# happykygo/GNN-eCommerce

Hardware: AMD Instinct MI355X
Metric: edges propagated/sec per LGConv layer (higher is better)
Workload: dtype f32; 1 GPU; configs[1]: 1639358 users x 54571 items, 20314816 directed edges, 3 LGConv layers, emb_dim 64, get_embedding (K hops + fused layer sum); parallelism=single, seed=0

## Files before the change

### gnn-ecommerce_amd/_native.py

```python
from __future__ import annotations

import ctypes
import os
from ctypes import CFUNCTYPE, POINTER, Structure, c_char_p, c_float, c_int, c_int32, c_int64, c_size_t, c_uint64, c_void_p
from typing import Optional

import torch

LIB_NAME = "liblgconv_hip.so"
LIB_PATH = os.environ.get("LGCN_LIB_PATH") or os.path.join(os.path.dirname(os.path.abspath(__file__)), "csrc", LIB_NAME)
ABI_VERSION = 14

ST_INDEX_OOB = 1
ST_SAMPLER_EXHAUSTED = 2

class SweepCfg(Structure):
    _fields_ = [("n_bands", c_int32), ("waves_per_band_round", c_int32), ("row_cap", c_int32), ("piece_cap", c_int32),
                ("lookahead", c_int32), ("groups", c_int32), ("round_order", c_int32)]


class SweepDims(Structure):
    _fields_ = [("n_bands", c_int32), ("rounds", c_int32), ("row_cap", c_int32), ("piece_cap", c_int32),
                ("n_rows", c_int32), ("groups", c_int32),
                ("n_waves", c_int64), ("n_slabs", c_int64), ("n_slots", c_int64), ("n_entries", c_int64),
# ... 71 lines not shown
    "lgc_sweep_dplan_free": (None, [c_void_p]),
    "lgc_sweep_ok": (c_int, [c_int32, c_int64, c_int64]),
    "lgc_spmm_sweep": (c_int, [c_void_p, c_void_p, c_void_p, c_void_p, c_int64, c_int32, c_int32, c_void_p, c_int32, c_void_p,
                               c_int32, c_void_p, c_int64, c_void_p, c_int64, c_void_p, c_int64, c_void_p, c_int64, c_float, c_float,
                               c_int32, c_void_p]),
    "lgc_apply_route": (c_int, [POINTER(OperatorC), c_int64, c_int64, c_int64, c_int64, c_int32]),
    "lgc_apply": (c_int, [POINTER(OperatorC), c_int64, c_void_p, c_int64, c_void_p, c_int64, c_void_p, c_int64, c_float, c_float,
                          c_int32, c_void_p]),
    "lgc_hop_exchange": (c_int, [POINTER(OperatorC), POINTER(OperatorC), c_int64, c_void_p, c_int64, c_void_p, c_int64, c_void_p,
                                 c_int64, c_float, c_float, c_int32, c_int32, c_int32, c_int32, EXCHANGE_FN, c_void_p, c_void_p]),
    "lgc_segment_sum": (c_int, [c_void_p, c_void_p, c_void_p, c_void_p, c_int64, c_float, c_void_p, c_int64, c_int64, c_int32,
                                c_int32, c_void_p]),
    "lgc_pair_dot_rows": (c_int, [c_void_p, c_int64, c_int32, c_int64, c_void_p, c_void_p, c_int64, c_void_p, c_void_p, c_void_p,
                                  c_void_p, c_void_p, c_void_p]),
    "lgc_reg_rows": (c_int, [c_void_p, c_int64, c_int32, c_int64, c_void_p, c_int64, c_void_p, c_int64, c_void_p, c_int64, c_float,
                             c_void_p, c_void_p, c_void_p, c_void_p]),
    "lgc_bpr_loss": (c_int, [c_void_p, c_void_p, c_int64, c_int64, c_void_p, c_void_p, c_void_p]),
    "lgc_pair_seed_vals": (c_int, [c_void_p, c_void_p, c_void_p, c_void_p, c_void_p, c_int64, c_int32, c_void_p, c_void_p]),
    "lgc_seed_prepare": (c_int, [c_void_p, c_int64, c_int64, c_int64, c_void_p, c_void_p, c_void_p, c_void_p, c_void_p, c_void_p,
                                 c_void_p, c_void_p, c_void_p]),
    "lgc_seed_flags": (c_int, [c_void_p, c_int64, c_int64, c_void_p, c_int32, c_void_p]),
    "lgc_seed_pull": (c_int, [c_void_p, c_void_p, c_int32, c_int32, c_int32, c_void_p, c_int32, c_void_p, c_int32, c_void_p,
                              c_void_p, c_void_p, c_void_p, c_void_p, c_int64, c_int64, c_void_p, c_int64, c_int32, c_void_p]),
    "lgc_seed_mark": (c_int, [c_void_p, c_void_p, c_int32, c_int32, c_void_p, c_int64, c_void_p, c_int64, c_int32, c_void_p]),
    "lgc_adam_step": (c_int, [c_void_p, c_void_p, c_void_p, c_void_p, c_int64, c_float, c_float, c_float, c_float, c_float,
                              c_float, c_void_p]),
    "lgc_adam_step_hp": (c_int, [c_void_p, c_void_p, c_void_p, c_void_p, c_int64, c_void_p, c_void_p]),
    "lgc_lincomb": (c_int, [c_void_p, c_int64, c_void_p, c_void_p, c_void_p, c_int32, c_int64, c_int32, c_void_p]),
    "lgc_mask_topk": (c_int, [c_void_p, c_int64, c_void_p, c_int64, c_void_p, c_void_p, c_void_p, c_int64, c_int32, c_int32,
                              c_void_p, c_void_p, c_void_p]),
    "lgc_fold_in": (c_int, [c_void_p, c_void_p, c_void_p, c_int64, c_void_p, c_void_p, c_int64, c_int64, c_void_p, c_void_p,
                            c_int64, c_int64, c_float, c_int32, c_int32, c_void_p, c_int64, c_void_p, c_void_p]),
    "lgc_score_rows": (c_int, [c_void_p, c_int64, c_int64, c_void_p, c_int64, c_void_p, c_int64, c_int32, c_int32, c_void_p,
                               c_int64, c_void_p, c_void_p]),
    "lgc_topk_hits": (c_int, [c_void_p, c_int64, c_int32, c_void_p, c_void_p, c_void_p, c_int64, c_int64, c_void_p, c_void_p,
                              c_void_p, c_void_p]),
    "lgc_metric_sums": (c_int, [c_void_p, c_void_p, c_int64, c_void_p, c_void_p, c_void_p]),
    "lgc_rank_metrics": (c_int, [c_void_p, c_int64, c_int32, c_void_p, c_void_p, c_void_p, c_void_p, c_int64, c_int64,
                                 POINTER(c_int32), c_int32, c_void_p, c_void_p, c_void_p, c_void_p, c_void_p]),
    "lgc_column_sums": (c_int, [c_void_p, c_int64, c_int64, c_int32, c_void_p, c_void_p]),
    "lgc_topk_coverage": (c_int, [c_void_p, c_int64, c_int32, c_int64, POINTER(c_int32), c_int32, c_int64, c_void_p, c_void_p,
                                  c_void_p, c_void_p]),
    "lgc_bfs_init": (c_int, [c_void_p, c_int32, c_int64, c_void_p, c_void_p, c_void_p, c_void_p]),
    "lgc_bfs_level": (c_int, [c_void_p, c_void_p, c_int32, c_int32, c_int32, c_void_p, c_int32, c_uint64, c_void_p, c_void_p,
                              c_void_p, c_void_p, c_void_p]),
    "lgc_bfs_resolve": (c_int, [c_void_p, c_void_p, c_int32, c_int64, c_int64, c_void_p, c_int32, c_void_p, c_void_p, c_void_p,
                                c_void_p]),
    "lgc_bfs_backtrack": (c_int, [c_void_p, c_void_p, c_int64, c_void_p, c_int32, c_void_p, c_void_p, c_int32, c_int64,
                                  c_void_p, c_int32, c_void_p]),
    "lgc_sample_triples": (c_int, [c_void_p, c_int64, c_void_p, c_void_p, c_void_p, c_void_p, c_int64, c_int64, c_uint64,
                                   c_uint64, c_void_p, c_void_p, c_void_p, c_void_p]),
    "lgc_pair_dot": (c_int, [c_void_p, c_int64, c_int32, c_int64, c_void_p, c_void_p, c_int64, c_void_p,
                             c_void_p, c_void_p]),
}


class NativeLibraryError(RuntimeError):
    """The HIP library is missing, stale, or a call into it failed."""


_lib: Optional[ctypes.CDLL] = None


def load() -> ctypes.CDLL:
    global _lib
    if _lib is not None:
        return _lib
    if not os.path.isfile(LIB_PATH):
        raise NativeLibraryError(
            f"{LIB_PATH} not found: the MI355X propagation library has not been built. "
            "Run `python -c 'import __graft_entry__ as g; g.build()'` (or `make -C gnn-ecommerce_amd/csrc`). "
            "There is no CPU or PyTorch fallback for this path.")
    try:
        lib = ctypes.CDLL(LIB_PATH)
    except OSError as exc:
        raise NativeLibraryError(f"cannot load {LIB_PATH}: {exc}") from exc
    for name, (restype, argtypes) in SIGNATURES.items():
        try:
            fn = getattr(lib, name)
        except AttributeError as exc:
            raise NativeLibraryError(f"{LIB_PATH} does not export {name}; rebuild it") from exc
        fn.restype, fn.argtypes = restype, argtypes
    if lib.lgc_abi_version() != ABI_VERSION:
        raise NativeLibraryError(f"{LIB_PATH} has ABI {lib.lgc_abi_version()}, expected {ABI_VERSION}; rebuild it")
    _lib = lib
    return lib


def check(code: int, what: str) -> None:
    if code != 0:
        text = load().lgc_error_string(code).decode()
        raise NativeLibraryError(f"{what} failed: {text} (code {code})")


def ptr(t: Optional[torch.Tensor]) -> Optional[int]:
    return None if t is None else t.data_ptr()


def stream_of(device: torch.device) -> int:
    return torch.cuda.current_stream(device).cuda_stream


def require_device(t: torch.Tensor, name: str) -> None:
    if not t.is_cuda:
        raise NativeLibraryError(
            f"{name} is on {t.device}: the LightGCN propagation path runs only on a ROCm device "
# ... 36 lines not shown
```

### gnn-ecommerce_amd/graph.py

```python
from __future__ import annotations

import os
from collections import OrderedDict
from dataclasses import dataclass, field
from typing import Dict, List, Optional, Tuple

import torch
from torch import Tensor

from . import _native

SHORT_MAX = int(os.environ.get("LGCN_SHORT_MAX", "32"))
CHUNK_LEN = int(os.environ.get("LGCN_CHUNK_LEN", "256"))
USER_CHUNK_LEN = int(os.environ.get("LGCN_USER_CHUNK_LEN", "4096"))
TILE_WIDTHS = (8, 16, 32)
USE_TILES = os.environ.get("LGCN_TILES", "1") == "1"
TILES_PER_WAVE = int(os.environ.get("LGCN_TILES_PER_WAVE", "1"))
TILE_ORDER = os.environ.get("LGCN_TILE_ORDER", "cold")
USE_SWEEP = os.environ.get("LGCN_SWEEP", "auto")
SWEEP_MIN_ENTRIES = int(os.environ.get("LGCN_SWEEP_MIN_ENTRIES", "1000000"))
SWEEP_ADAPTIVE_BANDS = os.environ.get("LGCN_SWEEP_ADAPTIVE_BANDS", "1") == "1"
SWEEP_PIECE_ENTRIES = int(os.environ.get("LGCN_SWEEP_PIECE_ENTRIES", "20"))
SWEEP_CFG = dict(n_bands=int(os.environ.get("LGCN_SWEEP_BANDS", "8")), waves_per_band_round=int(os.environ.get("LGCN_SWEEP_WAVES", "256")),
                 row_cap=int(os.environ.get("LGCN_SWEEP_ROW_CAP", "78")),
# ... 537 lines not shown

def _rows_split_scratch(device: torch.device, n_ids: int, dim: int) -> Tuple[Tensor, Tensor]:
    import threading
    key = (device, torch.cuda.current_stream(device).cuda_stream, threading.get_ident(), dim)
    got = _rows_scratch.get(key)
    if got is None or got[0].numel() < n_ids + 2:
        cap = max(n_ids, 4096)
        got = (torch.empty(cap + 2, dtype=torch.int32, device=device),
               torch.empty((cap + ROWS_SPLIT_ROOM, dim), dtype=torch.float32, device=device))
        _rows_scratch[key] = got
    return got


def apply_rows(op: "Operator", rows: Tensor, x: Tensor, out: Tensor, a: float = 1.0, r: Optional[Tensor] = None,
               b: float = 0.0, split: bool = False, compact: bool = False) -> Tensor:
    _check_table(x, "x")
    _check_table(out, "out")
    if r is not None:
        _check_table(r, "r")
    _native.require_device(rows, "rows")
    if rows.dtype != torch.int64 or rows.dim() != 1:
        raise TypeError("rows must be a 1-D int64 tensor")
    dim = x.size(1)
    if out.size(1) != dim or (r is not None and r.size(1) != dim):
        raise ValueError("x, out and r must have the same width")
    if compact and not split:
        raise ValueError("compact output needs split=True")
    rows = rows.contiguous()
    lib = _native.load()
    p = op.plan
    n_ids = rows.numel()
    with torch.cuda.device(x.device):
        if split:
            if n_ids == 0:
                return out
            if out.size(0) < (n_ids if compact else p.row_end):
                raise ValueError("out has too few rows")
            work, partials = _rows_split_scratch(x.device, n_ids, dim)
            code = lib.lgc_spmm_rows_split(_native.ptr(op.rowptr), _native.ptr(op.entries), p.row_begin, p.row_end, _native.ptr(rows),
                                           n_ids, x.size(0), _native.ptr(x), x.stride(0), _native.ptr(out), out.stride(0),
                                           out.size(0), _native.ptr(r), 0 if r is None else r.stride(0), float(a), float(b), dim,
                                           int(compact), _native.ptr(work), _native.ptr(partials), partials.size(0),
                                           _native.stream_of(x.device))
            _native.check(code, "lgc_spmm_rows_split")
            return out
        code = lib.lgc_spmm_rows(_native.ptr(op.rowptr), _native.ptr(op.entries), p.row_begin, p.row_end, _native.ptr(rows),
                                 n_ids, min(x.size(0), out.size(0)), _native.ptr(x), x.stride(0), _native.ptr(out),
                                 out.stride(0), _native.ptr(r), 0 if r is None else r.stride(0), float(a), float(b), dim,
                                 _native.stream_of(x.device))
    _native.check(code, "lgc_spmm_rows")
    return out


def sweep_choice(lib, dim: int, table_rows: int, stride: int) -> int:
    sweep = int(lib.lgc_sweep_ok(dim, table_rows, stride))
    return 0 if (sweep == 2 and not SWEEP_WIDE) else sweep


def _check_table(t: Tensor, name: str) -> None:
    _native.require_device(t, name)
    if t.dtype != torch.float32 or t.dim() != 2 or t.stride(1) != 1:
        raise TypeError(f"{name} must be a 2-D fp32 tensor with unit inner stride, got {t.dtype} {tuple(t.shape)}")


class PropGraph:

    def __init__(self, edge_index: Tensor, edge_weight: Optional[Tensor], num_nodes: int,
                 normalize: bool = True, short_max: int = SHORT_MAX, chunk_len: int = CHUNK_LEN,
                 keep_edge_values: bool = False):
        _native.require_device(edge_index, "edge_index")
        if edge_index.dtype != torch.int64 or edge_index.dim() != 2 or edge_index.size(0) != 2:
            raise TypeError("edge_index must be an int64 tensor of shape [2, E]")
        if edge_weight is not None:
            _native.require_device(edge_weight, "edge_weight")
            if edge_weight.dtype != torch.float32 or edge_weight.shape != (edge_index.size(1),):
                raise TypeError("edge_weight must be fp32 of shape [E]")
            if edge_weight.device != edge_index.device:
                raise RuntimeError("edge_index and edge_weight must be on the same device")
        self.device = edge_index.device
        self.num_nodes = int(num_nodes)
        self.num_edges = int(edge_index.size(1))
        self.normalize = bool(normalize)
        self.short_max, self.chunk_len = short_max, chunk_len
        self._key_refs = (edge_index, edge_weight)
        self._edge_index = edge_index.contiguous()
        self._edge_weight = None if edge_weight is None else edge_weight.contiguous()
        self.status = torch.zeros(4, dtype=torch.int32, device=self.device)
        self.deg = torch.empty(self.num_nodes, dtype=torch.float32, device=self.device)
        self.dis = torch.empty(self.num_nodes, dtype=torch.float32, device=self.device)
        self.edge_values = (torch.empty(self.num_edges, dtype=torch.float32, device=self.device)
                            if keep_edge_values else None)
        self.forward_op = self._build(by_source=False)
        self._transpose_op: Optional[Operator] = None
        self.split = self._find_bipartite_split()
        self._halves = {}

    def _build(self, by_source: bool, row_range: Optional[Tuple[int, int]] = None) -> Operator:
        lib = _native.load()
        n, e = self.num_nodes, self.num_edges
        ws_bytes = lib.lgc_build_workspace_bytes(n, e)
        if ws_bytes == 0:
            raise _native.NativeLibraryError("graph too large for int32 indexing")
        ws = torch.empty(ws_bytes, dtype=torch.uint8, device=self.device)
        rowptr = torch.empty(n + 1, dtype=torch.int32, device=self.device)
        entries = torch.empty((e, 2), dtype=torch.int32, device=self.device)
        first = not by_source
        with torch.cuda.device(self.device):
            code = lib.lgc_build_csr(
                _native.ptr(self._edge_index), _native.ptr(self._edge_weight), n, e,
                int(by_source), int(self.normalize),
                None if (first or not self.normalize) else _native.ptr(self.dis),
                _native.ptr(rowptr), _native.ptr(entries),
                _native.ptr(self.edge_values) if first else None,
                _native.ptr(self.deg) if first else None, _native.ptr(self.dis) if first else None,
                _native.ptr(ws), ws_bytes, _native.ptr(self.status), _native.stream_of(self.device))
        _native.check(code, "lgc_build_csr")
        if int(self.status[0].item()) & _native.ST_INDEX_OOB:
            raise IndexError(f"edge_index contains node ids outside [0, {n})")
        lo, hi = row_range if row_range is not None else (0, n)
        return Operator.build(n, rowptr, entries, lo, hi, self.short_max, self.chunk_len)

    def _find_bipartite_split(self) -> Optional[int]:
        if self.num_edges == 0:
            return None
        out = torch.empty(2, dtype=torch.int64, device=self.device)
        lib = _native.load()
        with torch.cuda.device(self.device):
            code = lib.lgc_bipartite_split(_native.ptr(self._edge_index), self.num_edges, _native.ptr(out),
                                           _native.stream_of(self.device))
        _native.check(code, "lgc_bipartite_split")
        lo, hi = out.tolist()
        return lo + 1 if lo < hi else None

    def halves(self, transpose: bool = False) -> Tuple[Operator, Operator]:
        if self.split is None:
            raise ValueError("graph is not bipartite")
        got = self._halves.get(transpose)
        if got is None:
            op = self.transpose_op if transpose else self.forward_op
            got = tuple(Operator.build(op.n_rows, op.rowptr, op.entries, lo, hi, self.short_max, chunk, sweep_cols=cols)
                        for (lo, hi), cols, chunk in (((0, self.split), (self.split, self.num_nodes),
                                                       max(self.chunk_len, USER_CHUNK_LEN)),
                                                      ((self.split, self.num_nodes), (0, self.split), self.chunk_len)))
            self._halves[transpose] = got
        return got

    def prepare(self, dim: int, table_rows: Optional[int] = None, transpose: bool = False) -> "PropGraph":
        lib = _native.load()
        rows = self.num_nodes if table_rows is None else int(table_rows)
        stride = dim if dim % 32 == 0 else (dim + 31) // 32 * 32
        ops = self.halves(transpose) if self.split is not None else ((self.transpose_op if transpose else self.forward_op),)
        import time
        for op in ops:
            t0 = time.perf_counter()
            if op.tiled and dim >= 4:
                op.tiles
            if PLAN_TIMING:
                torch.cuda.synchronize(self.device)
                print(f"[plan] rows [{op.plan.row_begin}, {op.plan.row_end}): tile classes {time.perf_counter() - t0:.3f} s", flush=True)
            t0 = time.perf_counter()
            if op.sweep_cols is not None:
                groups = sweep_choice(lib, dim, rows, stride)
                if groups:
                    op.sweep_plan(groups)
            if PLAN_TIMING:
                torch.cuda.synchronize(self.device)
                print(f"[plan] rows [{op.plan.row_begin}, {op.plan.row_end}): sweep plan total {time.perf_counter() - t0:.3f} s", flush=True)
        torch.cuda.synchronize(self.device)
        return self

    @property
    def transpose_op(self) -> Operator:
        if self._transpose_op is None:
            if self._edge_index is None:
                raise _native.NativeLibraryError("this graph was loaded from a file without its COO: the transposed "
                                                 "operator (backward pass) needs a graph built from edge_index")
            self._transpose_op = self._build(by_source=True)
        return self._transpose_op

    def save(self, path: str, extra: Optional[Dict[str, Tensor]] = None, meta: Optional[Dict[str, str]] = None) -> None:
        from safetensors.torch import save_file
        op = self.forward_op
        tensors = {"rowptr": op.rowptr, "entries": op.entries, "deg": self.deg, "dis": self.dis}
        for k, v in (extra or {}).items():
            tensors["extra." + k] = v
        meta = {**{"user." + k: str(v) for k, v in (meta or {}).items()},
                "format": "lgcn-graph-2", "num_nodes": str(self.num_nodes), "num_edges": str(self.num_edges),
                "normalize": str(int(self.normalize)), "split": "" if self.split is None else str(self.split)}
        save_file({k: v.detach().cpu().contiguous() for k, v in tensors.items()}, path, metadata=meta)

    @staticmethod
    def validate_csr(rowptr: Tensor, entries: Tensor, deg: Tensor, dis: Tensor, num_nodes: int, num_edges: int,
                     split: Optional[int], where: str) -> None:
        def bad(msg):
            raise ValueError(f"{where}: {msg}")
        if num_nodes < 0 or num_edges < 0 or num_nodes >= 2 ** 31 - 1 or num_edges >= 2 ** 31 - 1:
            bad("node or edge count out of range")
        if rowptr.dtype != torch.int32 or rowptr.shape != (num_nodes + 1,):
            bad(f"rowptr must be int32 [{num_nodes + 1}], got {rowptr.dtype} {tuple(rowptr.shape)}")
        if entries.dtype != torch.int32 or entries.shape != (num_edges, 2):
            bad(f"entries must be int32 [{num_edges}, 2], got {entries.dtype} {tuple(entries.shape)}")
        for name, t in (("deg", deg), ("dis", dis)):
            if t.dtype != torch.float32 or t.shape != (num_nodes,):
                bad(f"{name} must be fp32 [{num_nodes}], got {t.dtype} {tuple(t.shape)}")
        if split is not None and not 0 < split < num_nodes:
            bad(f"bipartite split {split} outside (0, {num_nodes})")
# ... 91 lines not shown
```

### gnn-ecommerce_amd/propagate.py

```python
from __future__ import annotations

import os
from typing import List, Optional, Sequence

import torch
from torch import Tensor
from torch.autograd.function import once_differentiable

from . import _native
from .graph import Operator, PropGraph, apply_rows


HOP_EVENT_LOG: Optional[list] = None


def _timed_apply(op: Operator, x: Tensor, out: Tensor, **kw) -> None:
    if HOP_EVENT_LOG is None:
        op.apply(x, out, **kw)
        return
    start, end = torch.cuda.Event(enable_timing=True), torch.cuda.Event(enable_timing=True)
    start.record()
    op.apply(x, out, **kw)
    end.record()
    HOP_EVENT_LOG.append((start, end))


def scratch_table(like: Tensor) -> Tensor:
    n, d = like.shape
    if PAD_INTERNAL and d % 32 != 0:
        stride = (d + 31) // 32 * 32
        return torch.empty((n, stride), dtype=like.dtype, device=like.device)[:, :d]
    return torch.empty_like(like)


PAD_INTERNAL = os.environ.get("LGCN_PAD_INTERNAL", "1") == "1"


def horner_hops(op: Operator, x0: Tensor, alphas: Sequence[float]) -> Tensor:
    k = len(alphas) - 1
    if k == 0:
        return x0 * alphas[0]
    x0 = x0.contiguous()
    h = torch.empty_like(x0) if k == 1 else scratch_table(x0)
    _timed_apply(op, x0, h, a=alphas[k], r=x0, b=alphas[k - 1])
    for layer in range(k - 2, -1, -1):
        nxt = torch.empty_like(x0) if layer == 0 else scratch_table(x0)
        _timed_apply(op, h, nxt, a=1.0, r=x0, b=alphas[layer])
        h = nxt
    return h


USE_BIPARTITE = os.environ.get("LGCN_BIPARTITE", "1") == "1"

class _HopSpan:

    def __enter__(self):
        self.log = HOP_EVENT_LOG
        if self.log is not None:
            self.start, self.end = torch.cuda.Event(enable_timing=True), torch.cuda.Event(enable_timing=True)
            self.start.record()
        return self

    def __exit__(self, *exc):
        if self.log is not None:
            self.end.record()
            self.log.append((self.start, self.end))


def bipartite_sum(user_op: Operator, item_op: Operator, split: int, x0: Tensor, alphas: Sequence[float],
                  final_rows: Optional[Tensor] = None) -> Tensor:
    k = len(alphas) - 1
    if k == 0:
        return x0 * alphas[0]
    x0 = x0.contiguous()
    n = x0.size(0)
    tables = [x0]
    uniform = UNIFORM_ALPHA_SHORTCUT and all(a == alphas[0] for a in alphas) and (UNIFORM_ALPHA_SHORTCUT == "force" or x0.size(1) % 32 == 0)
    for layer in range(1, k + 1):
        with _HopSpan():
            nxt = scratch_table(x0)
            if layer < k:
                item_op.apply(tables[-1], nxt)
                user_op.apply(tables[-1], nxt)
                tables.append(nxt)
            else:
                out = torch.empty_like(x0)
                rows_only = final_rows is not None
                if rows_only and SCORED_ITEM_ROWS_ONLY and item_op.listed_rows_pay(final_rows.numel()):
                    mix = nxt
                    _native.lincomb(mix[split:], [(alphas[l], tables[l - 1][split:]) for l in range(1, k + 1)])
                    if all(a == alphas[0] for a in alphas):
                        rest = mix
                    else:
                        rest = scratch_table(x0)
                        _native.lincomb(rest[split:], [(alphas[l], tables[l][split:]) for l in range(0, k)])
                    apply_rows(item_op, final_rows, tables[-1], out, a=alphas[k], r=rest, b=1.0, split=True)
                elif uniform:
                    mix = nxt
                    _native.lincomb(mix[split:], [(alphas[l], tables[l - 1][split:]) for l in range(1, k + 1)])
                    item_op.apply(tables[-1], out, a=alphas[k], r=mix, b=1.0)
                else:
                    item_op.apply(tables[-1], nxt)
                    tables.append(nxt)
                    mix = scratch_table(x0)
                    _native.lincomb(mix[split:], [(alphas[l], tables[l - 1][split:]) for l in range(1, k + 1)])
                    _native.lincomb(out[split:], [(alphas[l], tables[l][split:]) for l in range(0, k + 1)])
                if not rows_only:
                    user_op.apply(mix, out, a=1.0, r=x0, b=alphas[0])
                else:
                    apply_rows(user_op, final_rows, mix, out, a=1.0, r=x0, b=alphas[0])
    return out


def _layer_sum(graph: PropGraph, x: Tensor, alphas: tuple, transpose: bool, final_rows: Optional[Tensor] = None) -> Tensor:
    if USE_BIPARTITE and graph.split is not None and len(alphas) - 1 <= _native.MAX_TERMS - 1:
        user_op, item_op = graph.halves(transpose)
        return bipartite_sum(user_op, item_op, graph.split, x, alphas, final_rows if SCORED_ROWS_ONLY else None)
    return horner_hops(graph.transpose_op if transpose else graph.forward_op, x, alphas)


UNIFORM_ALPHA_SHORTCUT = {"0": False, "force": "force"}.get(os.environ.get("LGCN_UNIFORM_ALPHA_SHORTCUT", "1"), True)
SCORED_ROWS_ONLY = os.environ.get("LGCN_SCORED_ROWS_ONLY", "1") == "1"
SCORED_ITEM_ROWS_ONLY = os.environ.get("LGCN_SCORED_ITEM_ROWS_ONLY", "1") == "1"


class _PropagateSum(torch.autograd.Function):
    @staticmethod
    def forward(ctx, x0: Tensor, graph: PropGraph, alphas: tuple) -> Tensor:
        ctx.graph, ctx.alphas = graph, alphas
        return _layer_sum(graph, x0.detach(), alphas, transpose=False)

    @staticmethod
    @once_differentiable
    def backward(ctx, grad_out: Tensor):
        return _layer_sum(ctx.graph, grad_out.contiguous(), ctx.alphas, transpose=True), None, None


class _Hop(torch.autograd.Function):

    @staticmethod
    def forward(ctx, x: Tensor, graph: PropGraph) -> Tensor:
        ctx.graph = graph
        x = x.detach().contiguous()
        return graph.forward_op.apply(x, torch.empty_like(x))

    @staticmethod
    @once_differentiable
    def backward(ctx, grad_out: Tensor):
        g = grad_out.contiguous()
        return ctx.graph.transpose_op.apply(g, torch.empty_like(g)), None


def propagate_sum(x0: Tensor, graph: PropGraph, alphas: Sequence[float]) -> Tensor:
    _native.require_device(x0, "embedding table")
    return _PropagateSum.apply(x0, graph, tuple(float(a) for a in alphas))


def hop(x: Tensor, graph: PropGraph) -> Tensor:
    _native.require_device(x, "x")
    return _Hop.apply(x, graph)


_status_words = {}


def _status(device: torch.device) -> Tensor:
    t = _status_words.get(device)
    if t is None:
        t = torch.zeros(4, dtype=torch.int32, device=device)
        _status_words[device] = t
# ... 1001 lines not shown
```

### include/lgconv_hip.h

```cpp
#ifndef LGCONV_HIP_H
#define LGCONV_HIP_H

#include <stddef.h>
#include <stdint.h>

#ifdef __cplusplus
extern "C" {
#endif

#define LGC_ABI_VERSION 14

#define LGC_E_INVAL      (-1)
#define LGC_E_DIM        (-2)
#define LGC_E_WORKSPACE  (-3)
#define LGC_E_RANGE      (-4)
#define LGC_E_ALIGN      (-5)

#define LGC_ST_INDEX_OOB 1

typedef struct lgc_entry {
    int32_t col;
    float   val;
} lgc_entry;

// ... 215 lines not shown
                int32_t normalize, int32_t dim, float *out, int64_t out_stride, int32_t *status, void *stream);

int lgc_score_rows(const float *users, int64_t user_stride, int64_t n_user_rows, const int64_t *row_ids,
                   int64_t n_rows, const float *items, int64_t item_stride, int32_t n_items, int32_t dim,
                   float *out, int64_t out_stride, int32_t *status, void *stream);

int lgc_topk_hits(const int64_t *topk, int64_t topk_stride, int32_t k, const int64_t *pos_ptr,
                  const int64_t *pos_items, const int64_t *list_rows, int64_t n_rows, int64_t n_users,
                  int32_t *hits, double *recall, int32_t *status, void *stream);

int lgc_metric_sums(const int32_t *hits, const double *recall, int64_t n_rows, int64_t *hits_sum,
                    double *recall_sum, void *stream);

#define LGC_RM_PRECISION 0
#define LGC_RM_RECALL    1
#define LGC_RM_NDCG      2
#define LGC_RM_AP        3
#define LGC_RM_RR        4
#define LGC_RM_HIT       5
#define LGC_RM_COUNT     6
#define LGC_RM_MAX_CUTOFFS 8
int lgc_rank_metrics(const int64_t *topk, int64_t topk_stride, int32_t k, const int64_t *pos_ptr,
                     const int64_t *pos_items, const int64_t *pos_distinct, const int64_t *list_rows, int64_t n_rows,
                     int64_t n_users, const int32_t *cutoffs, int32_t n_cut, uint64_t *hit_bits, int32_t *hits,
                     double *metrics, int32_t *status, void *stream);

#define LGC_COLUMN_SUMS_MAX 64
int lgc_column_sums(const double *in, int64_t in_stride, int64_t n_rows, int32_t n_cols, double *out, void *stream);

int lgc_topk_coverage(const int64_t *topk, int64_t topk_stride, int32_t k, int64_t n_rows, const int32_t *cutoffs,
                      int32_t n_cut, int64_t n_items, uint32_t *bitmap, int64_t *counts, int32_t *status, void *stream);

#define LGC_BFS_MAX_SOURCES 64
#define LGC_BFS_UNSET (-3)
int lgc_bfs_init(const int64_t *sources, int32_t n_sources, int64_t n_nodes, uint64_t *seen, uint64_t *frontier,
                 int32_t *status, void *stream);
int lgc_bfs_level(const int32_t *rowptr, const lgc_entry *entries, int32_t row_begin, int32_t row_end, int32_t short_max,
                  const lgc_chunk *chunks, int32_t n_chunks, uint64_t active, const uint64_t *frontier_in,
                  uint64_t *frontier_out, uint64_t *seen, uint64_t *counters, void *stream);
int lgc_bfs_resolve(const int64_t *sources, const int64_t *targets, int32_t n_sources, int64_t n_targets, int64_t n_nodes,
                    const uint64_t *frontier, int32_t level, int32_t *dist, uint64_t *counters, int32_t *status,
                    void *stream);
int lgc_bfs_backtrack(const int32_t *rowptr, const lgc_entry *entries, int64_t n_nodes, const uint64_t *levels,
                      int32_t n_levels, const int64_t *targets, const int32_t *dist, int32_t n_sources, int64_t n_targets,
                      int64_t *paths, int32_t path_len, void *stream);

#define LGC_ST_SAMPLER_EXHAUSTED 2
int lgc_sample_triples(const int64_t *users, int64_t n,
                       const int32_t *pos_ptr, const int64_t *pos_items,
                       const int32_t *ign_ptr, const int64_t *ign_items,
                       int64_t n_users, int64_t n_items, uint64_t seed, uint64_t step,
                       int64_t *pos_out, int64_t *neg_out, int32_t *status, void *stream);

#ifdef __cplusplus
}
#endif
#endif
```

Before: 38.97 billion edges/s.

## Eliminate low-degree users via precomputed item-item Gram operator in bipartite propagation

```diff
diff --git a/gnn-ecommerce_amd/_native.py b/gnn-ecommerce_amd/_native.py
--- a/gnn-ecommerce_amd/_native.py
+++ b/gnn-ecommerce_amd/_native.py
@@ -147,6 +147,15 @@
                                    c_uint64, c_void_p, c_void_p, c_void_p, c_void_p]),
     "lgc_pair_dot": (c_int, [c_void_p, c_int64, c_int32, c_int64, c_void_p, c_void_p, c_int64, c_void_p,
                              c_void_p, c_void_p]),
+    "lgc_reduce_workspace_bytes": (c_size_t, [c_int64, c_int64]),
+    "lgc_reduce_count": (c_int, [c_void_p, c_void_p, c_int64, c_int64, c_int64, c_int32, c_void_p, c_size_t, c_void_p, c_void_p,
+                                 c_void_p]),
+    "lgc_reduce_fill": (c_int, [c_void_p, c_void_p, c_int64, c_int64, c_int64, c_void_p, c_void_p, c_int64, c_int64, c_void_p,
+                                c_void_p, c_void_p]),
+    "lgc_reduce_gram_workspace_bytes": (c_size_t, [c_int64]),
+    "lgc_reduce_gram_count": (c_int, [c_void_p, c_void_p, c_int64, c_int64, c_int64, c_void_p, c_int64, c_void_p, c_size_t,
+                                      c_void_p, c_void_p]),
+    "lgc_reduce_gram_fill": (c_int, [c_void_p, c_int64, c_int64, c_int64, c_int64, c_void_p, c_void_p, c_void_p]),
 }
 
 
diff --git a/gnn-ecommerce_amd/csrc/lgconv_reduce.hip b/gnn-ecommerce_amd/csrc/lgconv_reduce.hip
--- /dev/null
+++ b/gnn-ecommerce_amd/csrc/lgconv_reduce.hip
@@ -0,0 +1,362 @@
+#include "lgconv_common.h"
+
+#include <hipcub/hipcub.hpp>
+
+namespace {
+
+inline size_t r_align_up(size_t v, size_t a) { return (v + a - 1) / a * a; }
+
+struct ReduceWs {
+    int32_t *incount;
+    int32_t *keep_scan;
+    int32_t *ent_scan;
+    long long *pair_scan;
+    void *cub;
+    size_t cub_bytes;
+};
+
+size_t reduce_ws(void *base, int64_t n_nodes, int64_t n_edges, ReduceWs *ws) {
+    size_t cb32 = 0, cb64 = 0;
+    int32_t *n32 = nullptr;
+    long long *n64 = nullptr;
+    const int64_t longest = std::max<int64_t>(n_edges, n_nodes) + 1;
+    (void)hipcub::DeviceScan::ExclusiveSum(nullptr, cb32, n32, n32, (int)longest, (hipStream_t)0);
+    (void)hipcub::DeviceScan::ExclusiveSum(nullptr, cb64, n64, n64, (int)longest, (hipStream_t)0);
+    const size_t cb = std::max(cb32, cb64);
+    const uintptr_t p = reinterpret_cast<uintptr_t>(base);
+    size_t off = 0;
+    auto take = [&](size_t bytes) { const size_t at = off; off += r_align_up(bytes, 256); return p + at; };
+    const uintptr_t a_in = take((size_t)(n_nodes + 1) * 4), a_keep = take((size_t)(n_nodes + 1) * 4),
+                    a_ent = take((size_t)(n_edges + 1) * 4), a_pair = take((size_t)(n_edges + 1) * 8), a_cub = take(cb);
+    if (ws) {
+        ws->incount = reinterpret_cast<int32_t *>(a_in);
+        ws->keep_scan = reinterpret_cast<int32_t *>(a_keep);
+        ws->ent_scan = reinterpret_cast<int32_t *>(a_ent);
+        ws->pair_scan = reinterpret_cast<long long *>(a_pair);
+        ws->cub = reinterpret_cast<void *>(a_cub);
+        ws->cub_bytes = cb;
+    }
+    return off + 256;
+}
+
+struct GramWs {
+    unsigned long long *keys_in, *keys_out;
+    double *vals_in, *vals_out;
+    int32_t *head_scan;
+    void *cub;
+    size_t cub_bytes;
+};
+
+size_t gram_ws(void *base, int64_t n_pairs, GramWs *ws) {
+    size_t cb_sort = 0, cb_scan = 0;
+    unsigned long long *nk = nullptr;
+    double *nv = nullptr;
+    int32_t *n32 = nullptr;
+    const int64_t n = std::max<int64_t>(n_pairs, 1);
+    (void)hipcub::DeviceRadixSort::SortPairs(nullptr, cb_sort, nk, nk, nv, nv, (int)n, 0, 64, (hipStream_t)0);
+    (void)hipcub::DeviceScan::ExclusiveSum(nullptr, cb_scan, n32, n32, (int)(n + 1), (hipStream_t)0);
+    const size_t cb = std::max(cb_sort, cb_scan);
+    const uintptr_t p = reinterpret_cast<uintptr_t>(base);
+    size_t off = 0;
+    auto take = [&](size_t bytes) { const size_t at = off; off += r_align_up(bytes, 256); return p + at; };
+    const uintptr_t a_ki = take((size_t)n * 8), a_ko = take((size_t)n * 8), a_vi = take((size_t)n * 8), a_vo = take((size_t)n * 8),
+                    a_hs = take((size_t)(n + 1) * 4), a_cub = take(cb);
+    if (ws) {
+        ws->keys_in = reinterpret_cast<unsigned long long *>(a_ki);
+        ws->keys_out = reinterpret_cast<unsigned long long *>(a_ko);
+        ws->vals_in = reinterpret_cast<double *>(a_vi);
+        ws->vals_out = reinterpret_cast<double *>(a_vo);
+        ws->head_scan = reinterpret_cast<int32_t *>(a_hs);
+        ws->cub = reinterpret_cast<void *>(a_cub);
+        ws->cub_bytes = cb;
+    }
+    return off + 256;
+}
+
+__device__ inline int32_t row_of_entry(const int32_t *__restrict__ rowptr, int32_t n_rows, int32_t e) {
+    int32_t lo = 0, hi = n_rows;
+    while (hi - lo > 1) {
+        const int32_t mid = lo + (hi - lo) / 2;
+        if (rowptr[mid] <= e) lo = mid; else hi = mid;
+    }
+    return lo;
+}
+
+__global__ void k_reduce_incount(const int32_t *__restrict__ rowptr, const lgc_entry *__restrict__ entries, int32_t n_nodes,
+                                 int32_t split, int32_t n_edges, int32_t *__restrict__ incount) {
+    const int32_t e_begin = max(rowptr[split], 0), e_end = min(rowptr[n_nodes], n_edges);
+    for (int64_t e = e_begin + (int64_t)blockIdx.x * blockDim.x + threadIdx.x; e < e_end; e += (int64_t)gridDim.x * blockDim.x) {
+        const int32_t c = entries[e].col;
+        if (c >= 0 && c < split) atomicAdd(incount + c, 1);
+    }
+}
+
+__global__ void k_reduce_keep(const int32_t *__restrict__ rowptr, const int32_t *__restrict__ incount, int32_t split,
+                              int32_t max_deg, int32_t *__restrict__ keep) {
+    const int64_t u = (int64_t)blockIdx.x * blockDim.x + threadIdx.x;
+    if (u > split) return;
+    int32_t k = 0;
+    if (u < split) k = (rowptr[u + 1] - rowptr[u] <= max_deg && incount[u] <= max_deg) ? 0 : 1;
+    keep[u] = k;
+}
+
+__global__ void k_reduce_user_map(const int32_t *__restrict__ keep_scan, int32_t split, int32_t *__restrict__ user_map) {
+    const int64_t u = (int64_t)blockIdx.x * blockDim.x + threadIdx.x;
+    if (u >= split) return;
+    user_map[u] = keep_scan[u + 1] != keep_scan[u] ? keep_scan[u] : -1;
+}
+
+__global__ void k_reduce_entry_flags(const int32_t *__restrict__ rowptr, const lgc_entry *__restrict__ entries, int32_t n_nodes,
+                                     int32_t split, const int32_t *__restrict__ user_map, int32_t *__restrict__ ent_flag,
+                                     long long *__restrict__ pair_count, int32_t n_edges) {
+    const int64_t e = (int64_t)blockIdx.x * blockDim.x + threadIdx.x;
+    if (e > n_edges) return;
+    int32_t flag = 0;
+    long long pairs = 0;
+    if (e < n_edges) {
+        const int32_t row = row_of_entry(rowptr, n_nodes, (int32_t)e);
+        const int32_t c = entries[e].col;
+        if (row < split) {
+            flag = (user_map[row] >= 0 && c >= split && c < n_nodes) ? 1 : 0;
+        } else if (c >= 0 && c < split) {
+            if (user_map[c] >= 0) flag = 1;
+            else pairs = rowptr[c + 1] - rowptr[c];
+        }
+    }
+    ent_flag[e] = flag;
+    pair_count[e] = pairs;
+}
+
+__global__ void k_reduce_totals(const int32_t *__restrict__ rowptr, int32_t n_edges, int32_t split,
+                                const int32_t *__restrict__ keep_scan, const int32_t *__restrict__ ent_scan,
+                                const long long *__restrict__ pair_scan, long long *__restrict__ totals) {
+    if (blockIdx.x != 0 || threadIdx.x != 0) return;
+    totals[0] = keep_scan[split];
+    totals[1] = ent_scan[min(max(rowptr[split], 0), n_edges)];
+    totals[2] = ent_scan[n_edges];
+    totals[3] = pair_scan[n_edges];
+}
+
+__global__ void k_reduce_fill_rowptr(const int32_t *__restrict__ rowptr, int32_t n_nodes, int32_t split, int32_t n_h,
+                                     const int32_t *__restrict__ user_map, const int32_t *__restrict__ ent_scan,
+                                     int32_t n_edges, int32_t *__restrict__ rowptr_out) {
+    const int64_t r = (int64_t)blockIdx.x * blockDim.x + threadIdx.x;
+    if (r > n_nodes) return;
+    if (r == n_nodes) {
+        rowptr_out[n_h + (n_nodes - split)] = ent_scan[n_edges];
+        return;
+    }
+    const int32_t nr = r < split ? user_map[r] : n_h + ((int32_t)r - split);
+    if (nr >= 0 && nr < n_h + (n_nodes - split)) rowptr_out[nr] = ent_scan[min(max(rowptr[r], 0), n_edges)];
+}
+
+__global__ void k_reduce_fill_entries(const int32_t *__restrict__ rowptr, const lgc_entry *__restrict__ entries, int32_t n_nodes,
+                                      int32_t split, int32_t n_h, const int32_t *__restrict__ user_map,
+                                      const int32_t *__restrict__ ent_scan, int32_t n_edges, int32_t n_out,
+                                      lgc_entry *__restrict__ out) {
+    const int64_t e = (int64_t)blockIdx.x * blockDim.x + threadIdx.x;
+    if (e >= n_edges) return;
+    const int32_t dst = ent_scan[e];
+    if (ent_scan[e + 1] == dst || dst < 0 || dst >= n_out) return;
+    const int32_t row = row_of_entry(rowptr, n_nodes, (int32_t)e);
+    lgc_entry en = entries[e];
+    en.col = row < split ? en.col - (split - n_h) : user_map[en.col];
+    out[dst] = en;
+}
+
+__global__ void k_gram_expand(const int32_t *__restrict__ rowptr, const lgc_entry *__restrict__ entries, int32_t n_nodes,
+                              int32_t split, const long long *__restrict__ pair_scan, long long n_pairs,
+                              int32_t n_edges, unsigned long long *__restrict__ keys, double *__restrict__ vals) {
+    const int64_t e = (int64_t)max(rowptr[split], 0) + (int64_t)blockIdx.x * blockDim.x + threadIdx.x;
+    if (e >= n_edges) return;
+    const long long at = pair_scan[e], cnt = pair_scan[e + 1] - at;
+    if (cnt <= 0 || at < 0 || at + cnt > n_pairs) return;
+    const int32_t row = row_of_entry(rowptr, n_nodes, (int32_t)e);
+    const lgc_entry a = entries[e];
+    const int32_t s = rowptr[a.col];
+    if (s < 0 || s + cnt > n_edges) return;
+    long long w = at;
+    for (int32_t k = 0; k < cnt; ++k) {
+        const lgc_entry b = entries[s + k];
+        if (b.col < split || b.col >= n_nodes) continue;
+        keys[w] = ((unsigned long long)(uint32_t)(row - split) << 32) | (uint32_t)(b.col - split);
+        vals[w] = (double)a.val * (double)b.val;
+        ++w;
+    }
+}
+
+__global__ void k_gram_prefill(unsigned long long *__restrict__ keys, double *__restrict__ vals, long long n_pairs) {
+    const int64_t p = (int64_t)blockIdx.x * blockDim.x + threadIdx.x;
+    if (p >= n_pairs) return;
+    keys[p] = ~0ull;
+    vals[p] = 0.0;
+}
+
+__global__ void k_gram_heads(const unsigned long long *__restrict__ keys, long long n_pairs, int32_t *__restrict__ head) {
+    const int64_t p = (int64_t)blockIdx.x * blockDim.x + threadIdx.x;
+    if (p > n_pairs) return;
+    int32_t h = 0;
+    if (p < n_pairs && keys[p] != ~0ull) h = (p == 0 || keys[p] != keys[p - 1]) ? 1 : 0;
+    head[p] = h;
+}
+
+__global__ void k_gram_fill_entries(const unsigned long long *__restrict__ keys, const double *__restrict__ vals,
+                                    const int32_t *__restrict__ head_scan, long long n_pairs, int32_t n_h, int32_t n_out,
+                                    lgc_entry *__restrict__ out) {
+    const int64_t p = (int64_t)blockIdx.x * blockDim.x + threadIdx.x;
+    if (p >= n_pairs) return;
+    const int32_t dst = head_scan[p];
+    if (head_scan[p + 1] == dst || dst < 0 || dst >= n_out) return;
+    const unsigned long long key = keys[p];
+    double sum = 0.0;
+    for (int64_t q = p; q < n_pairs && keys[q] == key; ++q) sum += vals[q];
+    lgc_entry en;
+    en.col = n_h + (int32_t)(uint32_t)(key & 0xFFFFFFFFull);
+    en.val = (float)sum;
+    out[dst] = en;
+}
+
+__global__ void k_gram_fill_rowptr(const unsigned long long *__restrict__ keys, const int32_t *__restrict__ head_scan,
+                                   long long n_pairs, int32_t n_h, int32_t n_items, int32_t *__restrict__ rowptr_out) {
+    const int64_t r = (int64_t)blockIdx.x * blockDim.x + threadIdx.x;
+    if (r > (int64_t)n_h + n_items) return;
+    if (r <= n_h) {
+        rowptr_out[r] = 0;
+        return;
+    }
+    const unsigned long long want = (unsigned long long)(uint32_t)(r - n_h) << 32;
+    long long lo = 0, hi = n_pairs;
+    while (lo < hi) {
+        const long long mid = lo + (hi - lo) / 2;
+        if (keys[mid] < want) lo = mid + 1; else hi = mid;
+    }
+    rowptr_out[r] = head_scan[lo];
+}
+
+int reduce_args_ok(const int32_t *rowptr, const lgc_entry *entries, int64_t n_nodes, int64_t n_edges, int64_t split) {
+    if (n_nodes < 0 || n_edges < 0 || split < 0) return LGC_E_INVAL;
+    if (n_nodes >= INT32_MAX || n_edges >= INT32_MAX) return LGC_E_RANGE;
+    if (!rowptr || split <= 0 || split >= n_nodes || (n_edges > 0 && !entries)) return LGC_E_INVAL;
+    return 0;
+}
+
+}
+
+extern "C" {
+
+size_t lgc_reduce_workspace_bytes(int64_t n_nodes, int64_t n_edges) {
+    if (n_nodes < 0 || n_edges < 0 || n_nodes >= INT32_MAX || n_edges >= INT32_MAX) return 0;
+    return reduce_ws(nullptr, n_nodes, n_edges, nullptr);
+}
+
+int lgc_reduce_count(const int32_t *rowptr, const lgc_entry *entries, int64_t n_nodes, int64_t n_edges, int64_t split,
+                     int32_t max_deg, void *workspace, size_t workspace_bytes, int32_t *user_map, int64_t *totals,
+                     void *stream_) {
+    if (const int rc = reduce_args_ok(rowptr, entries, n_nodes, n_edges, split)) return rc;
+    if (max_deg < 0 || !workspace || !user_map || !totals) return LGC_E_INVAL;
+    if (workspace_bytes < lgc_reduce_workspace_bytes(n_nodes, n_edges)) return LGC_E_WORKSPACE;
+    if (reinterpret_cast<uintptr_t>(workspace) % 256 != 0) return LGC_E_ALIGN;
+    hipStream_t st = as_stream(stream_);
+    ReduceWs ws;
+    reduce_ws(workspace, n_nodes, n_edges, &ws);
+    const int32_t n = (int32_t)n_nodes, sp = (int32_t)split;
+    hipError_t err = hipMemsetAsync(ws.incount, 0, (size_t)(split + 1) * 4, st);
+    if (err != hipSuccess) return (int)err;
+    if (n_edges > 0)
+        hipLaunchKernelGGL(k_reduce_incount, dim3((unsigned)std::min<int64_t>(ceil_div(n_edges, kBlock), 256 * 16)), dim3(kBlock), 0,
+                           st, rowptr, entries, n, sp, (int32_t)n_edges, ws.incount);
+    hipLaunchKernelGGL(k_reduce_keep, dim3(ceil_div(split + 1, kBlock)), dim3(kBlock), 0, st, rowptr, ws.incount, sp, max_deg,
+                       ws.keep_scan);
+    err = hipcub::DeviceScan::ExclusiveSum(ws.cub, ws.cub_bytes, ws.keep_scan, ws.keep_scan, (int)(split + 1), st);
+    if (err != hipSuccess) return (int)err;
+    hipLaunchKernelGGL(k_reduce_user_map, dim3(ceil_div(split, kBlock)), dim3(kBlock), 0, st, ws.keep_scan, sp, user_map);
+    hipLaunchKernelGGL(k_reduce_entry_flags, dim3(ceil_div(n_edges + 1, kBlock)), dim3(kBlock), 0, st, rowptr, entries, n, sp,
+                       user_map, ws.ent_scan, ws.pair_scan, (int32_t)n_edges);
+    err = hipcub::DeviceScan::ExclusiveSum(ws.cub, ws.cub_bytes, ws.ent_scan, ws.ent_scan, (int)(n_edges + 1), st);
+    if (err != hipSuccess) return (int)err;
+    err = hipcub::DeviceScan::ExclusiveSum(ws.cub, ws.cub_bytes, ws.pair_scan, ws.pair_scan, (int)(n_edges + 1), st);
+    if (err != hipSuccess) return (int)err;
+    hipLaunchKernelGGL(k_reduce_totals, dim3(1), dim3(64), 0, st, rowptr, (int32_t)n_edges, sp, ws.keep_scan, ws.ent_scan, ws.pair_scan,
+                       reinterpret_cast<long long *>(totals));
+    return (int)hipGetLastError();
+}
+
+int lgc_reduce_fill(const int32_t *rowptr, const lgc_entry *entries, int64_t n_nodes, int64_t n_edges, int64_t split,
+                    const void *workspace, const int32_t *user_map, int64_t n_kept, int64_t n_out, int32_t *rowptr_out,
+                    lgc_entry *entries_out, void *stream_) {
+    if (const int rc = reduce_args_ok(rowptr, entries, n_nodes, n_edges, split)) return rc;
+    if (!workspace || !user_map || !rowptr_out || n_kept < 0 || n_kept > split || n_out < 0 || n_out > n_edges ||
+        (n_out > 0 && !entries_out))
+        return LGC_E_INVAL;
+    if (reinterpret_cast<uintptr_t>(workspace) % 256 != 0) return LGC_E_ALIGN;
+    hipStream_t st = as_stream(stream_);
+    ReduceWs ws;
+    reduce_ws(const_cast<void *>(workspace), n_nodes, n_edges, &ws);
+    const int32_t n = (int32_t)n_nodes, sp = (int32_t)split;
+    hipLaunchKernelGGL(k_reduce_fill_rowptr, dim3(ceil_div(n_nodes + 1, kBlock)), dim3(kBlock), 0, st, rowptr, n, sp,
+                       (int32_t)n_kept, user_map, ws.ent_scan, (int32_t)n_edges, rowptr_out);
+    if (n_out > 0)
+        hipLaunchKernelGGL(k_reduce_fill_entries, dim3(ceil_div(n_edges, kBlock)), dim3(kBlock), 0, st, rowptr, entries, n, sp,
+                           (int32_t)n_kept, user_map, ws.ent_scan, (int32_t)n_edges, (int32_t)n_out, entries_out);
+    return (int)hipGetLastError();
+}
+
+size_t lgc_reduce_gram_workspace_bytes(int64_t n_pairs) {
+    if (n_pairs < 0 || n_pairs >= INT32_MAX) return 0;
+    return gram_ws(nullptr, n_pairs, nullptr);
+}
+
+int lgc_reduce_gram_count(const int32_t *rowptr, const lgc_entry *entries, int64_t n_nodes, int64_t n_edges, int64_t split,
+                          const void *workspace, int64_t n_pairs, void *gram_workspace, size_t gram_workspace_bytes,
+                          int64_t *total, void *stream_) {
+    if (const int rc = reduce_args_ok(rowptr, entries, n_nodes, n_edges, split)) return rc;
+    if (n_pairs < 0 || !workspace || !total) return LGC_E_INVAL;
+    if (n_pairs >= INT32_MAX) return LGC_E_RANGE;
+    if (!gram_workspace) return LGC_E_INVAL;
+    if (gram_workspace_bytes < lgc_reduce_gram_workspace_bytes(n_pairs)) return LGC_E_WORKSPACE;
+    if (reinterpret_cast<uintptr_t>(workspace) % 256 != 0 || reinterpret_cast<uintptr_t>(gram_workspace) % 256 != 0) return LGC_E_ALIGN;
+    hipStream_t st = as_stream(stream_);
+    hipError_t err = hipMemsetAsync(total, 0, sizeof(int64_t), st);
+    if (err != hipSuccess) return (int)err;
+    if (n_pairs == 0) return 0;
+    ReduceWs ws;
+    reduce_ws(const_cast<void *>(workspace), n_nodes, n_edges, &ws);
+    GramWs gw;
+    gram_ws(gram_workspace, n_pairs, &gw);
+    const int32_t n = (int32_t)n_nodes, sp = (int32_t)split;
+    hipLaunchKernelGGL(k_gram_prefill, dim3(ceil_div(n_pairs, kBlock)), dim3(kBlock), 0, st, gw.keys_in, gw.vals_in,
+                       (long long)n_pairs);
+    hipLaunchKernelGGL(k_gram_expand, dim3(ceil_div(n_edges, kBlock)), dim3(kBlock), 0, st, rowptr, entries, n, sp, ws.pair_scan,
+                       (long long)n_pairs, (int32_t)n_edges, gw.keys_in, gw.vals_in);
+    err = hipcub::DeviceRadixSort::SortPairs(gw.cub, gw.cub_bytes, gw.keys_in, gw.keys_out, gw.vals_in, gw.vals_out, (int)n_pairs,
+                                             0, 64, st);
+    if (err != hipSuccess) return (int)err;
+    hipLaunchKernelGGL(k_gram_heads, dim3(ceil_div(n_pairs + 1, kBlock)), dim3(kBlock), 0, st, gw.keys_out, (long long)n_pairs,
+                       gw.head_scan);
+    err = hipcub::DeviceScan::ExclusiveSum(gw.cub, gw.cub_bytes, gw.head_scan, gw.head_scan, (int)(n_pairs + 1), st);
+    if (err != hipSuccess) return (int)err;
+    err = hipMemcpyAsync(total, gw.head_scan + n_pairs, sizeof(int32_t), hipMemcpyDeviceToDevice, st);
+    if (err != hipSuccess) return (int)err;
+    return (int)hipGetLastError();
+}
+
+int lgc_reduce_gram_fill(const void *gram_workspace, int64_t n_pairs, int64_t n_kept, int64_t n_items, int64_t n_out,
+                         int32_t *rowptr_out, lgc_entry *entries_out, void *stream_) {
+    if (n_pairs < 0 || n_kept < 0 || n_items < 1 || n_out < 0 || !rowptr_out) return LGC_E_INVAL;
+    if (n_pairs >= INT32_MAX || n_kept + n_items >= INT32_MAX) return LGC_E_RANGE;
+    if (n_out > n_pairs || (n_pairs > 0 && !gram_workspace) || (n_out > 0 && !entries_out)) return LGC_E_INVAL;
+    if (reinterpret_cast<uintptr_t>(gram_workspace) % 256 != 0) return LGC_E_ALIGN;
+    hipStream_t st = as_stream(stream_);
+    const int64_t rows = n_kept + n_items;
+    if (n_pairs == 0) return (int)hipMemsetAsync(rowptr_out, 0, (size_t)(rows + 1) * 4, st);
+    GramWs gw;
+    gram_ws(const_cast<void *>(gram_workspace), n_pairs, &gw);
+    hipLaunchKernelGGL(k_gram_fill_rowptr, dim3(ceil_div(rows + 1, kBlock)), dim3(kBlock), 0, st, gw.keys_out, gw.head_scan,
+                       (long long)n_pairs, (int32_t)n_kept, (int32_t)n_items, rowptr_out);
+    if (n_out > 0)
+        hipLaunchKernelGGL(k_gram_fill_entries, dim3(ceil_div(n_pairs, kBlock)), dim3(kBlock), 0, st, gw.keys_out, gw.vals_out,
+                           gw.head_scan, (long long)n_pairs, (int32_t)n_kept, (int32_t)n_out, entries_out);
+    return (int)hipGetLastError();
+}
+
+}
diff --git a/gnn-ecommerce_amd/graph.py b/gnn-ecommerce_amd/graph.py
--- a/gnn-ecommerce_amd/graph.py
+++ b/gnn-ecommerce_amd/graph.py
@@ -613,6 +613,94 @@
     return out
 
 
+ELIMINATE_MAX_DEG = os.environ.get("LGCN_ELIMINATE_MAX_DEG", "auto")
+ELIMINATE_AUTO_MAX_DEG = int(os.environ.get("LGCN_ELIMINATE_AUTO_MAX_DEG", "3"))
+ELIMINATE_MAX_GRAM_SHARE = float(os.environ.get("LGCN_ELIMINATE_MAX_GRAM_SHARE", "1.0"))
+GRAM_CHUNK_LEN = int(os.environ.get("LGCN_GRAM_CHUNK_LEN", "256"))
+
+
+@dataclass
+class ReducedCSR:
+    max_deg: int
+    n_h: int
+    n_items: int
+    user_map: Tensor
+    rowptr: Tensor
+    entries: Tensor
+    user_nnz: int
+    n_pairs: int
+    gram_rowptr: Tensor
+    gram_entries: Tensor
+
+    @property
+    def nnz(self) -> int:
+        return self.entries.size(0)
+
+    @property
+    def gram_nnz(self) -> int:
+        return self.gram_entries.size(0)
+
+
+def build_reduced_csr(rowptr: Tensor, entries: Tensor, split: int, num_nodes: int, max_deg: int) -> Optional[ReducedCSR]:
+    lib = _native.load()
+    _native.require_device(rowptr, "rowptr")
+    dev = rowptr.device
+    n_edges = entries.size(0)
+    n_items = num_nodes - split
+    u8 = dict(dtype=torch.uint8, device=dev)
+    i32 = dict(dtype=torch.int32, device=dev)
+    ws_bytes = lib.lgc_reduce_workspace_bytes(num_nodes, n_edges)
+    ws = torch.empty(max(ws_bytes, 1), **u8)
+    user_map = torch.empty(max(split, 1), **i32)
+    totals = torch.empty(4, dtype=torch.int64, device=dev)
+    args = (_native.ptr(rowptr), _native.ptr(entries), num_nodes, n_edges, split)
+    with torch.cuda.device(dev):
+        st = _native.stream_of(dev)
+        _native.check(lib.lgc_reduce_count(*args, int(max_deg), _native.ptr(ws), ws_bytes, _native.ptr(user_map),
+                                           _native.ptr(totals), st), "lgc_reduce_count")
+        n_h, user_nnz, nnz, n_pairs = totals.tolist()
+        rowptr_h = torch.empty(n_h + n_items + 1, **i32)
+        entries_h = torch.empty((nnz, 2), **i32)
+        _native.check(lib.lgc_reduce_fill(*args, _native.ptr(ws), _native.ptr(user_map), n_h, nnz, _native.ptr(rowptr_h),
+                                          _native.ptr(entries_h) if nnz else None, st), "lgc_reduce_fill")
+        gws_bytes = lib.lgc_reduce_gram_workspace_bytes(n_pairs)
+        if gws_bytes == 0:
+            return None
+        gws = torch.empty(gws_bytes, **u8)
+        total = torch.empty(1, dtype=torch.int64, device=dev)
+        code = lib.lgc_reduce_gram_count(*args, _native.ptr(ws), n_pairs, _native.ptr(gws), gws_bytes, _native.ptr(total), st)
+        if code == -4:
+            return None
+        _native.check(code, "lgc_reduce_gram_count")
+        gram_nnz = int(total.item())
+        gram_rowptr = torch.empty(n_h + n_items + 1, **i32)
+        gram_entries = torch.empty((gram_nnz, 2), **i32)
+        _native.check(lib.lgc_reduce_gram_fill(_native.ptr(gws), n_pairs, n_h, n_items, gram_nnz, _native.ptr(gram_rowptr),
+                                               _native.ptr(gram_entries) if gram_nnz else None, st), "lgc_reduce_gram_fill")
+    return ReducedCSR(int(max_deg), n_h, n_items, user_map[:split], rowptr_h, entries_h, user_nnz, n_pairs, gram_rowptr,
+                      gram_entries)
+
+
+@dataclass
+class ReducedGraph:
+    csr: ReducedCSR
+    n_h: int
+    offset: int
+    user_op_h: Optional[Operator]
+    item_op_h: Optional[Operator]
+    gram_op: Optional[Operator]
+
+    def nbytes(self) -> int:
+        c = self.csr
+        total = sum(t.numel() * 4 for t in (c.user_map, c.rowptr, c.entries, c.gram_rowptr, c.gram_entries))
+        for op in (self.user_op_h, self.item_op_h, self.gram_op):
+            if op is not None:
+                total += op.plan.chunks.numel() * 4 + sum(tc.slab.numel() * 4 + tc.order.numel() * 4 + tc.meta.numel() * 4
+                                                          for tc in (op._tiles or []))
+                total += sum(sw.nbytes() for sw in op._sweep.values())
+        return total
+
+
 def sweep_choice(lib, dim: int, table_rows: int, stride: int) -> int:
     sweep = int(lib.lgc_sweep_ok(dim, table_rows, stride))
     return 0 if (sweep == 2 and not SWEEP_WIDE) else sweep
@@ -706,13 +794,58 @@
             self._halves[transpose] = got
         return got
 
+    eliminate_max_deg: Optional[int] = None
+
+    def reduced(self, transpose: bool = False) -> Optional[ReducedGraph]:
+        if transpose or self.split is None:
+            return None
+        forced = self.eliminate_max_deg
+        auto = forced is None and ELIMINATE_MAX_DEG == "auto"
+        max_deg = int(forced) if forced is not None else (ELIMINATE_AUTO_MAX_DEG if auto else int(ELIMINATE_MAX_DEG))
+        if max_deg <= 0:
+            return None
+        key = ("reduced", max_deg, auto)
+        if key in self._halves:
+            return self._halves[key]
+        got = None
+        if not auto or self.halves(False)[1].sweep_cols is not None:
+            got = self._build_reduced(max_deg)
+            if got is not None and auto:
+                removed = self.forward_op.nnz - got.csr.nnz
+                if got.csr.gram_nnz > ELIMINATE_MAX_GRAM_SHARE * removed:
+                    got = None
+        self._halves[key] = got
+        return got
+
+    def _build_reduced(self, max_deg: int) -> Optional[ReducedGraph]:
+        op = self.forward_op
+        csr = build_reduced_csr(op.rowptr, op.entries, self.split, self.num_nodes, max_deg)
+        if csr is None:
+            return None
+        n_h, n_rows = csr.n_h, csr.n_h + csr.n_items
+        user_chunk = max(self.chunk_len, USER_CHUNK_LEN)
+        user_op_h = item_op_h = gram_op = None
+        if n_h > 0:
+            user_op_h = Operator.build(n_rows, csr.rowptr, csr.entries, 0, n_h, self.short_max, user_chunk,
+                                       sweep_cols=(n_h, n_rows))
+        if csr.nnz - csr.user_nnz > 0:
+            item_op_h = Operator.build(n_rows, csr.rowptr, csr.entries, n_h, n_rows, self.short_max, self.chunk_len,
+                                       sweep_cols=(0, n_h))
+        if csr.gram_nnz > 0:
+            gram_op = Operator.build(n_rows, csr.gram_rowptr, csr.gram_entries, n_h, n_rows, self.short_max, GRAM_CHUNK_LEN)
+        return ReducedGraph(csr, n_h, self.split - n_h, user_op_h, item_op_h, gram_op)
+
     def prepare(self, dim: int, table_rows: Optional[int] = None, transpose: bool = False) -> "PropGraph":
         lib = _native.load()
         rows = self.num_nodes if table_rows is None else int(table_rows)
         stride = dim if dim % 32 == 0 else (dim + 31) // 32 * 32
         ops = self.halves(transpose) if self.split is not None else ((self.transpose_op if transpose else self.forward_op),)
+        ops = [(op, rows) for op in ops]
+        red = self.reduced(transpose)
+        if red is not None:
+            ops += [(op, max(rows - red.offset, 0)) for op in (red.user_op_h, red.item_op_h, red.gram_op) if op is not None]
         import time
-        for op in ops:
+        for op, rows in ops:
             t0 = time.perf_counter()
             if op.tiled and dim >= 4:
                 op.tiles
diff --git a/gnn-ecommerce_amd/propagate.py b/gnn-ecommerce_amd/propagate.py
--- a/gnn-ecommerce_amd/propagate.py
+++ b/gnn-ecommerce_amd/propagate.py
@@ -68,20 +68,45 @@
 
 
 def bipartite_sum(user_op: Operator, item_op: Operator, split: int, x0: Tensor, alphas: Sequence[float],
-                  final_rows: Optional[Tensor] = None) -> Tensor:
+                  final_rows: Optional[Tensor] = None, reduced=None) -> Tensor:
     k = len(alphas) - 1
     if k == 0:
         return x0 * alphas[0]
     x0 = x0.contiguous()
     n = x0.size(0)
     tables = [x0]
+    red = reduced if k >= 2 else None
+    rows_items_only = final_rows is not None and SCORED_ITEM_ROWS_ONLY and item_op.listed_rows_pay(final_rows.numel()) \
+        if red is not None else False
+
+    def user_step(layer: int, x: Tensor, out_t: Tensor) -> None:
+        if red is None or (rows_items_only and layer == k - 1):
+            user_op.apply(x, out_t)
+        elif red.user_op_h is not None:
+            red.user_op_h.apply(x[red.offset:], out_t[red.offset:])
+
+    def item_step(layer: int, out_t: Tensor, a: float = 1.0, r: Optional[Tensor] = None) -> None:
+        o = red.offset
+        y = out_t[o:]
+        have = r is not None
+        if red.gram_op is not None:
+            red.gram_op.apply(tables[layer - 2][o:], y, a=a, r=r[o:] if have else None, b=1.0 if have else 0.0)
+        elif have:
+            _native.lincomb(out_t[split:], [(1.0, r[split:])])
+        else:
+            out_t[split:].zero_()
+        if red.item_op_h is not None:
+            red.item_op_h.apply(tables[layer - 1][o:], y, a=a, r=y, b=1.0)
     uniform = UNIFORM_ALPHA_SHORTCUT and all(a == alphas[0] for a in alphas) and (UNIFORM_ALPHA_SHORTCUT == "force" or x0.size(1) % 32 == 0)
     for layer in range(1, k + 1):
         with _HopSpan():
             nxt = scratch_table(x0)
             if layer < k:
-                item_op.apply(tables[-1], nxt)
-                user_op.apply(tables[-1], nxt)
+                if red is None or layer == 1:
+                    item_op.apply(tables[-1], nxt)
+                else:
+                    item_step(layer, nxt)
+                user_step(layer, tables[-1], nxt)
                 tables.append(nxt)
             else:
                 out = torch.empty_like(x0)
@@ -98,9 +123,15 @@
                 elif uniform:
                     mix = nxt
                     _native.lincomb(mix[split:], [(alphas[l], tables[l - 1][split:]) for l in range(1, k + 1)])
-                    item_op.apply(tables[-1], out, a=alphas[k], r=mix, b=1.0)
+                    if red is None:
+                        item_op.apply(tables[-1], out, a=alphas[k], r=mix, b=1.0)
+                    else:
+                        item_step(k, out, a=alphas[k], r=mix)
                 else:
-                    item_op.apply(tables[-1], nxt)
+                    if red is None:
+                        item_op.apply(tables[-1], nxt)
+                    else:
+                        item_step(k, nxt)
                     tables.append(nxt)
                     mix = scratch_table(x0)
                     _native.lincomb(mix[split:], [(alphas[l], tables[l - 1][split:]) for l in range(1, k + 1)])
@@ -115,7 +146,8 @@
 def _layer_sum(graph: PropGraph, x: Tensor, alphas: tuple, transpose: bool, final_rows: Optional[Tensor] = None) -> Tensor:
     if USE_BIPARTITE and graph.split is not None and len(alphas) - 1 <= _native.MAX_TERMS - 1:
         user_op, item_op = graph.halves(transpose)
-        return bipartite_sum(user_op, item_op, graph.split, x, alphas, final_rows if SCORED_ROWS_ONLY else None)
+        return bipartite_sum(user_op, item_op, graph.split, x, alphas, final_rows if SCORED_ROWS_ONLY else None,
+                             reduced=graph.reduced(transpose) if len(alphas) > 2 else None)
     return horner_hops(graph.transpose_op if transpose else graph.forward_op, x, alphas)
 
 
diff --git a/include/lgconv_hip.h b/include/lgconv_hip.h
--- a/include/lgconv_hip.h
+++ b/include/lgconv_hip.h
@@ -291,6 +291,20 @@
                        int64_t n_users, int64_t n_items, uint64_t seed, uint64_t step,
                        int64_t *pos_out, int64_t *neg_out, int32_t *status, void *stream);
 
+size_t lgc_reduce_workspace_bytes(int64_t n_nodes, int64_t n_edges);
+int lgc_reduce_count(const int32_t *rowptr, const lgc_entry *entries, int64_t n_nodes, int64_t n_edges, int64_t split,
+                     int32_t max_deg, void *workspace, size_t workspace_bytes, int32_t *user_map, int64_t *totals,
+                     void *stream);
+int lgc_reduce_fill(const int32_t *rowptr, const lgc_entry *entries, int64_t n_nodes, int64_t n_edges, int64_t split,
+                    const void *workspace, const int32_t *user_map, int64_t n_kept, int64_t n_out, int32_t *rowptr_out,
+                    lgc_entry *entries_out, void *stream);
+size_t lgc_reduce_gram_workspace_bytes(int64_t n_pairs);
+int lgc_reduce_gram_count(const int32_t *rowptr, const lgc_entry *entries, int64_t n_nodes, int64_t n_edges, int64_t split,
+                          const void *workspace, int64_t n_pairs, void *gram_workspace, size_t gram_workspace_bytes,
+                          int64_t *total, void *stream);
+int lgc_reduce_gram_fill(const void *gram_workspace, int64_t n_pairs, int64_t n_kept, int64_t n_items, int64_t n_out,
+                         int32_t *rowptr_out, lgc_entry *entries_out, void *stream);
+
 #ifdef __cplusplus
 }
 #endif
```

After: 39.97 billion edges/s (median of 6 runs). 2.6% higher.
